# waldstein94/Stratified-Transformer

Measured on AMD Instinct MI355X. Metric: points/sec through StratifiedAttention fwd+bwd, 100k-pt scene, higher is better.
Workload: dtype f32

## Files before the change

### stratified_transformer_amd/csrc/cell_attn.hip

```cpp
#include "cell_common.h"

namespace p2 {


typedef unsigned short bf16_t;
__device__ __forceinline__ float4 ld_row4(const float *p) { return *reinterpret_cast<const float4 *>(p); }
__device__ __forceinline__ float4 ld_row4(const bf16_t *p) {
    const uint2 u = *reinterpret_cast<const uint2 *>(p);
    return make_float4(__uint_as_float(u.x << 16), __uint_as_float(u.x & 0xffff0000u), __uint_as_float(u.y << 16), __uint_as_float(u.y & 0xffff0000u));
}
__device__ __forceinline__ float ld_elem(const float *p) { return *p; }
__device__ __forceinline__ float ld_elem(const bf16_t *p) { return __uint_as_float((unsigned)*p << 16); }
template <typename T>
__device__ __forceinline__ void stage_table_t(T *lds, const T *__restrict__ tab, int L, int h, int head) {
    const int total = 3 * L * 16;
    for (int x = threadIdx.x; x < total; x += blockDim.x) {
        const int i = x % 16, r = (x / 16) % L, ax = x / (16 * L);
        lds[x] = tab[(((size_t)r * h + head) * 16 + i) * 3 + ax];
    }
}

template <int LCAP>
struct TabGeo {
    static constexpr int TS = 3 * LCAP * 16;
    static constexpr size_t bytes(size_t elem) { return (size_t)3 * TS * elem; }
};
struct RowOff {
    int o0, o1, o2;
};
__device__ __forceinline__ RowOff row_off(unsigned w, int L, int c) {
    RowOff r;
    r.o0 = (int)(w & 255u) * 16 + 4 * c;
    r.o1 = (int)(L + ((w >> 8) & 255u)) * 16 + 4 * c;
    r.o2 = (int)(2 * L + ((w >> 16) & 255u)) * 16 + 4 * c;
    return r;
}
template <int OFF>
__device__ __forceinline__ float4 tsum_at(const float *lds, RowOff r) {
    return add4(add4(*reinterpret_cast<const float4 *>(lds + OFF + r.o0), *reinterpret_cast<const float4 *>(lds + OFF + r.o1)),
                *reinterpret_cast<const float4 *>(lds + OFF + r.o2));
}

struct Rows3 {
    float4 a, b, c;
};
template <int OFF, typename T>
__device__ __forceinline__ Rows3 rows_at(const T *lds, RowOff r) {
    Rows3 x;
    x.a = ld_row4(lds + OFF + r.o0);
    x.b = ld_row4(lds + OFF + r.o1);
    x.c = ld_row4(lds + OFF + r.o2);
    return x;
}
typedef float f32x2c __attribute__((ext_vector_type(2)));
__device__ __forceinline__ float4 padd4(float4 a, float4 b) {
    const f32x2c lo = f32x2c{a.x, a.y} + f32x2c{b.x, b.y}, hi = f32x2c{a.z, a.w} + f32x2c{b.z, b.w};
    return make_float4(lo.x, lo.y, hi.x, hi.y);
}
__device__ __forceinline__ float4 pfma4(float s, float4 a, float4 acc) {
    const f32x2c ss = f32x2c{s, s};
    const f32x2c lo = __builtin_elementwise_fma(ss, f32x2c{a.x, a.y}, f32x2c{acc.x, acc.y});
    const f32x2c hi = __builtin_elementwise_fma(ss, f32x2c{a.z, a.w}, f32x2c{acc.z, acc.w});
    return make_float4(lo.x, lo.y, hi.x, hi.y);
}
__device__ __forceinline__ float4 rsum(Rows3 r) { return padd4(padd4(r.a, r.b), r.c); }
__device__ __forceinline__ f32x2c pdot_acc(float4 a, float4 b, f32x2c acc) {
    acc = __builtin_elementwise_fma(f32x2c{a.x, a.y}, f32x2c{b.x, b.y}, acc);
    return __builtin_elementwise_fma(f32x2c{a.z, a.w}, f32x2c{b.z, b.w}, acc);
}
__device__ __forceinline__ float pdot4(float4 a, float4 b) {
    const f32x2c r = pdot_acc(a, b, f32x2c{0.f, 0.f});
    return r.x + r.y;
}

template <int NPMAX, typename F>
__device__ __forceinline__ void dispatch_passes(int np, F f) {
    if (np <= 2) f(std::integral_constant<int, 2>{});
    else if (np == 3) f(std::integral_constant<int, 3>{});
    else if (np == 4 || NPMAX <= 4) f(std::integral_constant<int, 4>{});
    else if constexpr (NPMAX > 4) {
        if (np <= 6) f(std::integral_constant<int, 6>{});
        else f(std::integral_constant<int, 8>{});
    }
}

template <typename T>
struct LaneCtx {
    const T *lds;
    int L, lane, p, c, head, h, C, hoff;
};
struct CellBufs {
    rsrc_t rel, key, qid;
};

template <int NPA, typename T>
__device__ __forceinline__ void load_key_rows(const LaneCtx<T> &x, const CellBufs &cb, const T *__restrict__ rows, int j0, float4 (&r4)[NPA]) {
    unsigned keys[NPA];
    bload_words<NPA>(cb.key, (j0 + x.p * NPA) * 4, keys);
#pragma unroll
    for (int t = 0; t < NPA; t++) r4[t] = ld_row4(rows + (size_t)keys[t] * x.C + x.hoff);
}

template <int NPA, int TS, typename T>
__device__ __forceinline__ void fwd_sweep_logits(const LaneCtx<T> &x, const CellTask &ct, const CellBufs &cb, rsrc_t rs_p,
                                                 const T *__restrict__ q, const T *__restrict__ k, float *__restrict__ ml,
                                                 int ch, bool single, int j0, int nkc) {
    const int p = x.p, c = x.c;
    const int nvalid = min(max(nkc - p * NPA, 0), NPA);
    float4 k4[NPA];
    load_key_rows<NPA, T>(x, cb, k, j0, k4);
    int ids = (int)bload_u32(cb.qid, x.lane * 4);
    int i_nx = __builtin_amdgcn_readlane(ids, 0);
    float4 q4_nx = ld_row4(q + (size_t)i_nx * x.C + x.hoff);
    unsigned w_nx[NPA];
    bload_words<NPA>(cb.rel, (j0 + p * NPA) * 4, w_nx);
    for (int il = 0; il < ct.nq; il++) {
        const int i = i_nx;
        const float4 q4 = q4_nx;
        unsigned w[NPA];
#pragma unroll
        for (int t = 0; t < NPA; t++) w[t] = w_nx[t];
        const int roff = (il * ct.nk + j0 + p * NPA) * 4;
        if (((il + 1) & 63) == 0) ids = (int)bload_u32(cb.qid, (il + 1 + x.lane) * 4);
        i_nx = __builtin_amdgcn_readlane(ids, (il + 1) & 63);
        q4_nx = ld_row4(q + (size_t)i_nx * x.C + x.hoff);
        bload_words<NPA>(cb.rel, roff + ct.nk * 4, w_nx);
        float lg[NPA];
        float mx = -INFINITY;
        RowOff ro = row_off(w[0], x.L, c);
        Rows3 rq = rows_at<0, T>(x.lds, ro), rk = rows_at<TS, T>(x.lds, ro);
#pragma unroll
        for (int t = 0; t < NPA; t++) {
            Rows3 rq1 = rq, rk1 = rk;
            if (t + 1 < NPA) {
                ro = row_off(w[t + 1], x.L, c);
                rq1 = rows_at<0, T>(x.lds, ro);
                rk1 = rows_at<TS, T>(x.lds, ro);
            }
            const f32x2c d2 = pdot_acc(k4[t], rsum(rk), pdot_acc(q4, rsum(rq), pdot_acc(q4, k4[t], f32x2c{0.f, 0.f})));
            const float s = quad_sum(d2.x + d2.y);
            lg[t] = (t < nvalid && !(w[t] >> 31)) ? s : -INFINITY;
            mx = fmaxf(mx, lg[t]);
            rq = rq1;
            rk = rk1;
            __builtin_amdgcn_sched_barrier(0);
        }
        mx = slots_max16(mx);
        if (single) {
            float sum = 0.f;
#pragma unroll
            for (int t = 0; t < NPA; t++) {
                lg[t] = __expf(lg[t] - mx);
                sum += lg[t];
            }
            const float inv = 1.0f / slots_sum16(sum);
#pragma unroll
            for (int t = 0; t < NPA; t++) lg[t] *= inv;
            if (c == 0) bstore_floats<NPA>(rs_p, roff, lg, nvalid);
        } else {
            float *st = ml + ((size_t)i * x.h + x.head) * 2;
            const float m_old = ch ? st[0] : -INFINITY, l_old = ch ? st[1] : 0.f;
            const float m_new = fmaxf(m_old, mx);
            float sum = 0.f;
#pragma unroll
            for (int t = 0; t < NPA; t++) sum += __expf(lg[t] - m_new);
            if (c == 0) bstore_floats<NPA>(rs_p, roff, lg, nvalid);
            sum = slots_sum16(sum);
            if (x.lane == 0) {
                st[0] = m_new;
                st[1] = (m_old == -INFINITY ? 0.f : l_old * __expf(m_old - m_new)) + sum;
            }
        }
    }
}

template <int NPA, int TS, typename T>
__device__ __forceinline__ void fwd_sweep_values(const LaneCtx<T> &x, const CellTask &ct, const CellBufs &cb, rsrc_t rs_p,
                                                 const T *__restrict__ v, const float *__restrict__ ml, float *__restrict__ out,
                                                 int ch, bool single, int j0, int nkc) {
    const int p = x.p, c = x.c;
    const int nvalid = min(max(nkc - p * NPA, 0), NPA);
    float4 v4[NPA];
    load_key_rows<NPA, T>(x, cb, v, j0, v4);
    unsigned w_nx[NPA];
    float a_nx[NPA];
    bload_words<NPA>(cb.rel, (j0 + p * NPA) * 4, w_nx);
    bload_floats<NPA>(rs_p, (j0 + p * NPA) * 4, a_nx);
    int ids = (int)bload_u32(cb.qid, x.lane * 4);
    for (int il = 0; il < ct.nq; il++) {
        if (il && (il & 63) == 0) ids = (int)bload_u32(cb.qid, (il + x.lane) * 4);
        const int i = __builtin_amdgcn_readlane(ids, il & 63);
        const int roff = (il * ct.nk + j0 + p * NPA) * 4;
        unsigned w[NPA];
        float a[NPA];
#pragma unroll
        for (int t = 0; t < NPA; t++) {
            w[t] = w_nx[t];
            a[t] = a_nx[t];
        }
        bload_words<NPA>(cb.rel, roff + ct.nk * 4, w_nx);
        bload_floats<NPA>(rs_p, roff + ct.nk * 4, a_nx);
        if (!single) {
            const float *st = ml + ((size_t)i * x.h + x.head) * 2;
            const float m = st[0], inv = 1.0f / st[1];
#pragma unroll
            for (int t = 0; t < NPA; t++) a[t] = __expf(a[t] - m) * inv;
            if (c == 0) bstore_floats<NPA>(rs_p, roff, a, nvalid);
        }
        float4 acc = make_float4(0.f, 0.f, 0.f, 0.f);
        Rows3 rv = rows_at<2 * TS, T>(x.lds, row_off(w[0], x.L, c));
#pragma unroll
        for (int t = 0; t < NPA; t++) {
            Rows3 rv1 = rv;
            if (t + 1 < NPA) rv1 = rows_at<2 * TS, T>(x.lds, row_off(w[t + 1], x.L, c));
            const float at = t < nvalid ? a[t] : 0.f;
            acc = pfma4(at, padd4(rsum(rv), v4[t]), acc);
            rv = rv1;
            __builtin_amdgcn_sched_barrier(0);
        }
        const float4 tot = slots_sum16_4(acc);
        if (p == 0) {
            float *o = out + (size_t)i * x.C + x.hoff;
            stg4(o, ch ? add4(tot, ldg4(o)) : tot);
        }
    }
}

template <int NP, int LCAP, typename T>
__global__ __launch_bounds__(CA_WAVES * 64) void cell_fwd_kernel(pointops2_cell_plan pl, int h, int L, const T *__restrict__ q,
                                                                 const T *__restrict__ k, const T *__restrict__ v,
                                                                 const T *__restrict__ table_q, const T *__restrict__ table_k,
                                                                 const T *__restrict__ table_v, float *__restrict__ out,
                                                                 float *__restrict__ ml, float *__restrict__ pbuf, size_t plane) {
    constexpr int D = 16, TS = TabGeo<LCAP>::TS;
    extern __shared__ float lds_raw[];
    T *lds = reinterpret_cast<T *>(lds_raw);
    LaneCtx<T> x;
    x.lds = lds;
    x.L = L;
    x.h = h;
    x.head = blockIdx.y;
    x.C = h * D;
    x.lane = threadIdx.x & 63;
    x.p = x.lane >> 2;
    x.c = x.lane & 3;
    x.hoff = x.head * D + 4 * x.c;
    const int wave = __builtin_amdgcn_readfirstlane(threadIdx.x >> 6);
    stage_table_t<T>(lds, table_q, L, h, x.head);
    stage_table_t<T>(lds + TS, table_k, L, h, x.head);
    stage_table_t<T>(lds + 2 * TS, table_v, L, h, x.head);
    __syncthreads();
    const int nC = share_count(pl, pl.counts[0]);
    float *pb = pbuf + (size_t)x.head * plane;
    const int slots = gridDim.x * CA_WAVES, slot = blockIdx.x * CA_WAVES + wave;
    for (int round = 0; round * slots < nC; round++) {
        const int task = snake_task(round, slot, slots);
        if (task >= nC) continue;
        const CellTask ct = cell_task(pl, share_task(pl, task));
        const int nch = (ct.nk + 16 * NP - 1) / (16 * NP);
        const unsigned tile_bytes = (unsigned)ct.nq * ct.nk * 4u;
        CellBufs cb;
        cb.rel = make_rsrc(pl.relp + ct.pbase, tile_bytes);
        cb.key = make_rsrc(pl.cell_keys + ct.kb, (unsigned)ct.nk * 4u);
        cb.qid = make_rsrc(pl.cell_order + ct.qs, (unsigned)ct.nq * 4u);
        const rsrc_t rs_p = make_rsrc(pb + ct.pbase, tile_bytes);
        for (int ch = 0; ch < nch; ch++) {
            const int j0 = ch * 16 * NP, nkc = min(16 * NP, ct.nk - j0);
            dispatch_passes<NP>((nkc + 15) >> 4, [&](auto tag) {
                fwd_sweep_logits<decltype(tag)::value, TS, T>(x, ct, cb, rs_p, q, k, ml, ch, nch == 1, j0, nkc);
            });
        }
        for (int ch = 0; ch < nch; ch++) {
            const int j0 = ch * 16 * NP, nkc = min(16 * NP, ct.nk - j0);
            dispatch_passes<NP>((nkc + 15) >> 4, [&](auto tag) {
                fwd_sweep_values<decltype(tag)::value, TS, T>(x, ct, cb, rs_p, v, ml, out, ch, nch == 1, j0, nkc);
            });
        }
    }
}

template <int NPA, typename T>
__device__ __forceinline__ void flush_key_pass(float *scr, float4 acc, rsrc_t rs_key, int j0, int t, int nkc, float *__restrict__ grad,
                                               const LaneCtx<T> &x) {
    *reinterpret_cast<float4 *>(scr + x.p * 16 + 4 * x.c) = acc;
    __builtin_amdgcn_s_waitcnt(0xC07F);
    __builtin_amdgcn_wave_barrier();
#pragma unroll
    for (int kk = 0; kk < 4; kk++) {
        const int s = (x.lane >> 4) + 4 * kk;
        const int jl = s * NPA + t;
        const int key = (int)bload_u32(rs_key, (j0 + jl) * 4);
        if (jl < nkc) unsafeAtomicAdd(grad + (size_t)key * x.C + x.head * 16 + (x.lane & 15), scr[s * 16 + (x.lane & 15)]);
    }
    __builtin_amdgcn_s_waitcnt(0xC07F);
    __builtin_amdgcn_wave_barrier();
}

template <int NPA, int TS, typename T>
__device__ __forceinline__ void bwd_sweep_values(const LaneCtx<T> &x, const CellTask &ct, const CellBufs &cb, rsrc_t rs_p, rsrc_t rs_g,
                                                 float *scr, const float *__restrict__ go, const float *__restrict__ out,
                                                 const T *__restrict__ v, float *__restrict__ grad_v, int j0, int nkc) {
    const int p = x.p, c = x.c;
    const int nvalid = min(max(nkc - p * NPA, 0), NPA);
    float4 v4[NPA], dv4[NPA];
    load_key_rows<NPA, T>(x, cb, v, j0, v4);
#pragma unroll
    for (int t = 0; t < NPA; t++) dv4[t] = make_float4(0.f, 0.f, 0.f, 0.f);
    unsigned w_nx[NPA];
    float a_nx[NPA];
    bload_words<NPA>(cb.rel, (j0 + p * NPA) * 4, w_nx);
    bload_floats<NPA>(rs_p, (j0 + p * NPA) * 4, a_nx);
    int ids = (int)bload_u32(cb.qid, x.lane * 4);
    int i_nx = __builtin_amdgcn_readlane(ids, 0);
    float4 go_nx = ldg4(go + (size_t)i_nx * x.C + x.hoff), o_nx = ldg4(out + (size_t)i_nx * x.C + x.hoff);
    for (int il = 0; il < ct.nq; il++) {
        const int roff = (il * ct.nk + j0 + p * NPA) * 4;
        const float4 go4 = go_nx, o4 = o_nx;
        unsigned w[NPA];
        float a[NPA];
#pragma unroll
        for (int t = 0; t < NPA; t++) {
            w[t] = w_nx[t];
            a[t] = t < nvalid ? a_nx[t] : 0.f;
        }
        if (((il + 1) & 63) == 0) ids = (int)bload_u32(cb.qid, (il + 1 + x.lane) * 4);
        i_nx = __builtin_amdgcn_readlane(ids, (il + 1) & 63);
        go_nx = ldg4(go + (size_t)i_nx * x.C + x.hoff);
        o_nx = ldg4(out + (size_t)i_nx * x.C + x.hoff);
        bload_words<NPA>(cb.rel, roff + ct.nk * 4, w_nx);
        bload_floats<NPA>(rs_p, roff + ct.nk * 4, a_nx);
        const float delta = quad_sum(pdot4(go4, o4));
        float gs[NPA];
        Rows3 rv = rows_at<2 * TS, T>(x.lds, row_off(w[0], x.L, c));
#pragma unroll
        for (int t = 0; t < NPA; t++) {
            Rows3 rv1 = rv;
            if (t + 1 < NPA) rv1 = rows_at<2 * TS, T>(x.lds, row_off(w[t + 1], x.L, c));
            const float ga = quad_sum(pdot4(go4, padd4(rsum(rv), v4[t])));
            gs[t] = a[t] * (ga - delta);
            dv4[t] = pfma4(a[t], go4, dv4[t]);
            rv = rv1;
            __builtin_amdgcn_sched_barrier(0);
        }
        if (c == 0) bstore_floats<NPA>(rs_g, roff, gs, nvalid);
    }
#pragma unroll
    for (int t = 0; t < NPA; t++) flush_key_pass<NPA, T>(scr, dv4[t], cb.key, j0, t, nkc, grad_v, x);
}

template <int NPA, int TS, typename T>
__device__ __forceinline__ void bwd_sweep_keys(const LaneCtx<T> &x, const CellTask &ct, const CellBufs &cb, rsrc_t rs_g, float *scr,
                                               const T *__restrict__ q, const T *__restrict__ k, float *__restrict__ grad_q,
                                               float *__restrict__ grad_k, int ch, int j0, int nkc) {
    const int p = x.p, c = x.c;
    const int nvalid = min(max(nkc - p * NPA, 0), NPA);
    float4 k4[NPA], dk4[NPA];
    load_key_rows<NPA, T>(x, cb, k, j0, k4);
#pragma unroll
    for (int t = 0; t < NPA; t++) dk4[t] = make_float4(0.f, 0.f, 0.f, 0.f);
    unsigned w_nx[NPA];
    float g_nx[NPA];
    bload_words<NPA>(cb.rel, (j0 + p * NPA) * 4, w_nx);
    bload_floats<NPA>(rs_g, (j0 + p * NPA) * 4, g_nx);
    int ids = (int)bload_u32(cb.qid, x.lane * 4);
    int i_nx = __builtin_amdgcn_readlane(ids, 0);
    float4 q_nx = ld_row4(q + (size_t)i_nx * x.C + x.hoff);
    for (int il = 0; il < ct.nq; il++) {
        const int i = i_nx;
        const int roff = (il * ct.nk + j0 + p * NPA) * 4;
        const float4 q4 = q_nx;
        unsigned w[NPA];
        float g[NPA];
#pragma unroll
        for (int t = 0; t < NPA; t++) {
            w[t] = w_nx[t];
            g[t] = t < nvalid ? g_nx[t] : 0.f;
        }
        if (((il + 1) & 63) == 0) ids = (int)bload_u32(cb.qid, (il + 1 + x.lane) * 4);
        i_nx = __builtin_amdgcn_readlane(ids, (il + 1) & 63);
        q_nx = ld_row4(q + (size_t)i_nx * x.C + x.hoff);
        bload_words<NPA>(cb.rel, roff + ct.nk * 4, w_nx);
        bload_floats<NPA>(rs_g, roff + ct.nk * 4, g_nx);
        float4 dq = make_float4(0.f, 0.f, 0.f, 0.f);
        RowOff ro = row_off(w[0], x.L, c);
        Rows3 rq = rows_at<0, T>(x.lds, ro), rk = rows_at<TS, T>(x.lds, ro);
#pragma unroll
        for (int t = 0; t < NPA; t++) {
            Rows3 rq1 = rq, rk1 = rk;
            if (t + 1 < NPA) {
                ro = row_off(w[t + 1], x.L, c);
                rq1 = rows_at<0, T>(x.lds, ro);
                rk1 = rows_at<TS, T>(x.lds, ro);
            }
            dq = pfma4(g[t], padd4(rsum(rq), k4[t]), dq);
            dk4[t] = pfma4(g[t], padd4(rsum(rk), q4), dk4[t]);
            rq = rq1;
            rk = rk1;
            __builtin_amdgcn_sched_barrier(0);
        }
        const float4 tot = slots_sum16_4(dq);
        if (p == 0) {
            float *o = grad_q + (size_t)i * x.C + x.hoff;
            stg4(o, ch ? add4(tot, ldg4(o)) : tot);
        }
    }
#pragma unroll
    for (int t = 0; t < NPA; t++) flush_key_pass<NPA, T>(scr, dk4[t], cb.key, j0, t, nkc, grad_k, x);
}

template <int NP, int LCAP, typename T>
__global__ __launch_bounds__(CA_WAVES_BWD * 64) void cell_bwd_kernel(pointops2_cell_plan pl, int h, int L, const float *__restrict__ go,
                                                                 const T *__restrict__ q, const T *__restrict__ k,
                                                                 const T *__restrict__ v, const float *__restrict__ out,
                                                                 const T *__restrict__ table_q, const T *__restrict__ table_k,
                                                                 const T *__restrict__ table_v, const float *__restrict__ pbuf,
                                                                 float *__restrict__ gsbuf, size_t plane, float *__restrict__ grad_q,
                                                                 float *__restrict__ grad_k, float *__restrict__ grad_v) {
    constexpr int D = 16, TS = TabGeo<LCAP>::TS;
    extern __shared__ float lds_raw[];
    T *lds = reinterpret_cast<T *>(lds_raw);
    LaneCtx<T> x;
    x.lds = lds;
    x.L = L;
    x.h = h;
    x.head = blockIdx.y;
    x.C = h * D;
    x.lane = threadIdx.x & 63;
    x.p = x.lane >> 2;
    x.c = x.lane & 3;
    x.hoff = x.head * D + 4 * x.c;
    const int wave = __builtin_amdgcn_readfirstlane(threadIdx.x >> 6);
    float *scr = reinterpret_cast<float *>(lds + 3 * TS) + wave * 256;
    stage_table_t<T>(lds, table_q, L, h, x.head);
    stage_table_t<T>(lds + TS, table_k, L, h, x.head);
    stage_table_t<T>(lds + 2 * TS, table_v, L, h, x.head);
    __syncthreads();
    const int nC = share_count(pl, pl.counts[0]);
    const float *pb = pbuf + (size_t)x.head * plane;
    float *gb = gsbuf + (size_t)x.head * plane;
    const int slots = gridDim.x * CA_WAVES_BWD, slot = blockIdx.x * CA_WAVES_BWD + wave;
    for (int round = 0; round * slots < nC; round++) {
        const int task = snake_task(round, slot, slots);
        if (task >= nC) continue;
        const CellTask ct = cell_task(pl, share_task(pl, task));
        const int nch = (ct.nk + 16 * NP - 1) / (16 * NP);
        const unsigned tile_bytes = (unsigned)ct.nq * ct.nk * 4u;
        CellBufs cb;
        cb.rel = make_rsrc(pl.relp + ct.pbase, tile_bytes);
        cb.key = make_rsrc(pl.cell_keys + ct.kb, (unsigned)ct.nk * 4u);
        cb.qid = make_rsrc(pl.cell_order + ct.qs, (unsigned)ct.nq * 4u);
        const rsrc_t rs_p = make_rsrc(pb + ct.pbase, tile_bytes);
        const rsrc_t rs_g = make_rsrc(gb + ct.pbase, tile_bytes);
        for (int ch = 0; ch < nch; ch++) {
            const int j0 = ch * 16 * NP, nkc = min(16 * NP, ct.nk - j0);
            dispatch_passes<NP>((nkc + 15) >> 4, [&](auto tag) {
                bwd_sweep_values<decltype(tag)::value, TS, T>(x, ct, cb, rs_p, rs_g, scr, go, out, v, grad_v, j0, nkc);
            });
        }
        for (int ch = 0; ch < nch; ch++) {
            const int j0 = ch * 16 * NP, nkc = min(16 * NP, ct.nk - j0);
            dispatch_passes<NP>((nkc + 15) >> 4, [&](auto tag) {
                bwd_sweep_keys<decltype(tag)::value, TS, T>(x, ct, cb, rs_g, scr, q, k, grad_q, grad_k, ch, j0, nkc);
            });
        }
    }
}

struct CFixScale {
    float mul, inv;
};
__device__ __forceinline__ CFixScale c_row_scale(unsigned maxbits, int n) {
    CFixScale sc;
    if (maxbits >= 0x7f800000u) {
        sc.mul = 0.f;
        sc.inv = __uint_as_float(0x7fc00000u);
        return sc;
    }
    const int E = (int)(maxbits >> 23) - 126;
    const int bits_n = 32 - __clz(max(n, 1));
    const int S = max(-126, min(126, 30 - bits_n - E));
    sc.mul = __uint_as_float((unsigned)(S + 127) << 23);
    sc.inv = __uint_as_float((unsigned)(127 - S) << 23);
    return sc;
}

constexpr int CT_WAVES = 8;

template <int TA>
struct CellTableGeo {
    static constexpr int LP = TA * 16;
    static constexpr int ROW = 3 * LP + 16;
    static constexpr size_t walk_bytes() { return (size_t)CT_WAVES * 4 * ROW * 4; }
    static constexpr size_t sum_bytes() { return (size_t)LP * 48 * 4; }
    static constexpr size_t lds_bytes() { return walk_bytes() > sum_bytes() ? walk_bytes() : sum_bytes(); }
};

template <int TA, bool BYKEY, typename XT>
__device__ __forceinline__ void cell_table_grad_body(const pointops2_cell_plan &pl, int h, int L, const float *__restrict__ wbuf, size_t plane,
                                                     const XT *__restrict__ X, float *__restrict__ grad_table) {
    constexpr int D = 16;
    constexpr int MAXP = BYKEY ? 4 : 8;
    using G = CellTableGeo<TA>;
    extern __shared__ float lds[];
    const int wave = __builtin_amdgcn_readfirstlane(threadIdx.x >> 6), lane = threadIdx.x & 63;
    const int C = h * D, head = blockIdx.y;
    const int p = lane >> 2, c = lane & 3;
    const int kq = lane >> 4, col = lane & 15;
    int *hist = reinterpret_cast<int *>(lds) + wave * 4 * G::ROW;
    const float *wb = wbuf + (size_t)head * plane;

    f32x4c acc[TA][3];
#pragma unroll
    for (int bt = 0; bt < TA; bt++)
#pragma unroll
        for (int ax = 0; ax < 3; ax++) acc[bt][ax] = f32x4c{0.f, 0.f, 0.f, 0.f};
    for (int x = lane; x < 4 * G::ROW; x += 64) hist[x] = 0;

    const int nC = BYKEY ? pl.counts[4] : share_count(pl, pl.counts[0]);
    const int slots = gridDim.x * CT_WAVES, slot = blockIdx.x * CT_WAVES + wave;
    for (int round = 0; round * slots < nC; round++) {
        const int task = snake_task(round, slot, slots);
        if (task >= nC) continue;
        CellTask ct;
        if (BYKEY) {
            const int c0 = __builtin_amdgcn_readfirstlane(pl.parent_first[task]), c1 = __builtin_amdgcn_readfirstlane(pl.parent_first[task + 1]);
            ct.qs = __builtin_amdgcn_readfirstlane(pl.cell_qstart[c0]);
            ct.nq = __builtin_amdgcn_readfirstlane(pl.cell_qstart[c1]) - ct.qs;
            ct.kb = __builtin_amdgcn_readfirstlane(pl.cell_kbase[c0]);
            ct.nk = __builtin_amdgcn_readfirstlane(pl.cell_kbase[c0 + 1]) - ct.kb;
            ct.pbase = __builtin_amdgcn_readfirstlane(pl.cell_pbase[c0]);
        } else {
            ct = cell_task(pl, share_task(pl, task));
        }
        const unsigned tile_bytes = (unsigned)ct.nq * ct.nk * 4u;
        const rsrc_t rs_rel = make_rsrc(pl.relp + ct.pbase, tile_bytes);
        const rsrc_t rs_w = make_rsrc(wb + ct.pbase, tile_bytes);
        const rsrc_t rs_row = BYKEY ? make_rsrc(pl.cell_keys + ct.kb, (unsigned)ct.nk * 4u) : make_rsrc(pl.cell_order + ct.qs, (unsigned)ct.nq * 4u);
        const int nrows = BYKEY ? ct.nk : ct.nq, nent = BYKEY ? ct.nq : ct.nk;
        auto entry_off = [&](int r0, int ent) -> int { return (BYKEY ? ent * ct.nk + r0 + c : (r0 + c) * ct.nk + ent) * 4; };
        auto consume = [&](int r0, int e0, float xv, unsigned (&wr)[MAXP], float (&wt)[MAXP]) {
            const int ne = min(nent - e0, 16 * MAXP);
            const bool row_ok = r0 + c < nrows;
            unsigned mxb = 0u;
#pragma unroll
            for (int t = 0; t < MAXP; t++) {
                const bool live = row_ok && e0 + 16 * t + p < nent && !(wr[t] >> 31);
                wt[t] = live ? wt[t] : 0.f;
                mxb = max(mxb, __float_as_uint(fabsf(wt[t])));
            }
            const CFixScale sc = c_row_scale(wave_max_u32(mxb), ne);
            int *myh = hist + c * G::ROW;
#pragma unroll
            for (int t = 0; t < MAXP; t++) {
                if (16 * t < ne && wt[t] != 0.f) {
                    const int v = __float2int_rn(wt[t] * sc.mul);
                    atomicAdd(&myh[wr[t] & 255u], v);
                    atomicAdd(&myh[G::LP + ((wr[t] >> 8) & 255u)], v);
                    atomicAdd(&myh[2 * G::LP + ((wr[t] >> 16) & 255u)], v);
                }
            }
            __builtin_amdgcn_s_waitcnt(0xC07F);
            __builtin_amdgcn_wave_barrier();
            const float b = xv * sc.inv;
#pragma unroll
            for (int bt = 0; bt < TA; bt++)
#pragma unroll
                for (int ax = 0; ax < 3; ax++) {
                    const float a = (float)__hip_atomic_exchange(&hist[kq * G::ROW + ax * G::LP + bt * 16 + col], 0, __ATOMIC_RELAXED,
                                                                 __HIP_MEMORY_SCOPE_WORKGROUP);
                    acc[bt][ax] = __builtin_amdgcn_mfma_f32_16x16x4f32(a, b, acc[bt][ax], 0, 0, 0);
                }
            __builtin_amdgcn_s_waitcnt(0xC07F);
            __builtin_amdgcn_wave_barrier();
        };
        unsigned wr_n[MAXP];
        float wt_n[MAXP];
#pragma unroll
        for (int t = 0; t < MAXP; t++) {
            wr_n[t] = 0x80000000u;
            wt_n[t] = 0.f;
            if (16 * t < nent) {
                wr_n[t] = bload_u32(rs_rel, entry_off(0, 16 * t + p));
                wt_n[t] = bload_f32(rs_w, entry_off(0, 16 * t + p));
            }
        }
        int pt_n = (int)bload_u32(rs_row, kq * 4);
        float xv_n = ld_elem(X + (size_t)pt_n * C + head * D + col);
        pt_n = (int)bload_u32(rs_row, (4 + kq) * 4);
        for (int r0 = 0; r0 < nrows; r0 += 4) {
            unsigned wr[MAXP];
            float wt[MAXP];
#pragma unroll
            for (int t = 0; t < MAXP; t++) {
                wr[t] = wr_n[t];
                wt[t] = wt_n[t];
            }
            const float xv = r0 + kq < nrows ? xv_n : 0.f;
            xv_n = ld_elem(X + (size_t)pt_n * C + head * D + col);
            pt_n = (int)bload_u32(rs_row, (r0 + 8 + kq) * 4);
#pragma unroll
            for (int t = 0; t < MAXP; t++)
                if (16 * t < nent) {
                    wr_n[t] = bload_u32(rs_rel, entry_off(r0 + 4, 16 * t + p));
                    wt_n[t] = bload_f32(rs_w, entry_off(r0 + 4, 16 * t + p));
                }
            consume(r0, 0, xv, wr, wt);
            for (int e0 = 16 * MAXP; e0 < nent; e0 += 16 * MAXP) {
#pragma unroll
                for (int t = 0; t < MAXP; t++) {
                    wr[t] = bload_u32(rs_rel, entry_off(r0, e0 + 16 * t + p));
                    wt[t] = bload_f32(rs_w, entry_off(r0, e0 + 16 * t + p));
                }
                consume(r0, e0, xv, wr, wt);
            }
        }
    }
    __syncthreads();
    float *sum = lds;
    for (int w = 0; w < CT_WAVES; w++) {
        if (wave == w) {
#pragma unroll
            for (int bt = 0; bt < TA; bt++)
#pragma unroll
                for (int ax = 0; ax < 3; ax++)
#pragma unroll
                    for (int reg = 0; reg < 4; reg++) {
                        float *d = &sum[((bt * 16 + kq * 4 + reg) * 16 + col) * 3 + ax];
                        *d = w ? *d + acc[bt][ax][reg] : acc[bt][ax][reg];
                    }
        }
        __syncthreads();
    }
    for (int x = threadIdx.x; x < L * 48; x += CT_WAVES * 64) {
        const float val = sum[x];
        if (val != 0.f) unsafeAtomicAdd(grad_table + ((size_t)(x / 48) * h + head) * 48 + x % 48, val);
    }
}

template <int TA, typename T>
__global__ __launch_bounds__(CT_WAVES * 64) void cell_table_grad3_kernel(pointops2_cell_plan pl, int h, int L, const float *__restrict__ gsbuf,
                                                                         const float *__restrict__ pbuf, size_t plane,
                                                                         const T *__restrict__ q, const T *__restrict__ k,
                                                                         const float *__restrict__ grad_out, float *__restrict__ gtq,
                                                                         float *__restrict__ gtk, float *__restrict__ gtv) {
    if (blockIdx.z == 0) cell_table_grad_body<TA, true, T>(pl, h, L, gsbuf, plane, k, gtk);
    else if (blockIdx.z == 1) cell_table_grad_body<TA, false, T>(pl, h, L, gsbuf, plane, q, gtq);
    else cell_table_grad_body<TA, false, float>(pl, h, L, pbuf, plane, grad_out, gtv);
}

static int cell_fwd_variant(const pointops2_cell_plan *plan, int h, int hdim, int L, bool bf16, const char **why) {
    *why = nullptr;
    if (plan == nullptr || plan->n_points <= 0) return POINTOPS2_CELL_FWD_NONE;
    if (hdim != 16) { *why = "cell_attention: d != 16"; return POINTOPS2_CELL_FWD_ERROR; }
    if (L < 1) { *why = "cell_attention: no table rows"; return POINTOPS2_CELL_FWD_ERROR; }
    if (L != plan->table_rows) { *why = "cell_attention: the tables' row count differs from the plan's table_rows"; return POINTOPS2_CELL_FWD_ERROR; }
    if (L > 160) { *why = "cell_attention: more than 160 table rows (use the operators)"; return POINTOPS2_CELL_FWD_ERROR; }
    if (L > 80) return POINTOPS2_CELL_FWD_VALU160;
    if (!bf16) {
        const double avg_queries = (double)plan->n_pairs / (double)(plan->n_keyslots > 0 ? plan->n_keyslots : 1);
        if (!((long long)plan->n_points * h >= 96000 && avg_queries < 15.0)) return L <= 64 ? POINTOPS2_CELL_FWD_MFMA64 : POINTOPS2_CELL_FWD_MFMA80;
    }
    return POINTOPS2_CELL_FWD_VALU80;
}

template <typename T>
static void launch_cell_fwd(hipStream_t st, const pointops2_cell_plan *plan, int h, int hdim, int L, const T *q, const T *k, const T *v, const T *table_q,
                            const T *table_k, const T *table_v, float *out, float *ml, float *pbuf) {
    const char *why;
    const int variant = cell_fwd_variant(plan, h, hdim, L, !std::is_same<T, float>::value, &why);
    if (why != nullptr) { set_error(why); return; }
    if (variant == POINTOPS2_CELL_FWD_NONE) return;
    if constexpr (std::is_same<T, float>::value) {
        if (variant == POINTOPS2_CELL_FWD_MFMA64 || variant == POINTOPS2_CELL_FWD_MFMA80) {
            cell_fwd_mfma_launch(st, variant, plan, h, L, q, k, v, table_q, table_k, table_v, out, pbuf);
            check_launch();
            return;
        }
    }
    const dim3 block(CA_WAVES * 64);
    const size_t plane = (size_t)plan->n_pairs;
    if (variant == POINTOPS2_CELL_FWD_VALU80) {
        const size_t lds = TabGeo<80>::bytes(sizeof(T));
        allow_big_lds(cell_fwd_kernel<CA_NP, 80, T>, lds);
        const dim3 grid(cell_grid_x(1, plan->n_cells, h, CA_WAVES), h);
        hipLaunchKernelGGL((cell_fwd_kernel<CA_NP, 80, T>), grid, block, lds, st, *plan, h, L, q, k, v, table_q, table_k, table_v, out, ml,
                           pbuf, plane);
    } else {
        const size_t lds = TabGeo<160>::bytes(sizeof(T));
        allow_big_lds(cell_fwd_kernel<CA_NP, 160, T>, lds);
        const dim3 grid(cell_grid_x(1, plan->n_cells, h, CA_WAVES), h);
        hipLaunchKernelGGL((cell_fwd_kernel<CA_NP, 160, T>), grid, block, lds, st, *plan, h, L, q, k, v, table_q, table_k, table_v, out, ml,
                           pbuf, plane);
    }
    check_launch();
}

template <typename T>
static void launch_cell_bwd(hipStream_t st, const pointops2_cell_plan *plan, int h, int hdim, int L, const float *grad_out, const T *q, const T *k, const T *v,
                            const float *out, const T *table_q, const T *table_k, const T *table_v, const float *pbuf, float *gsbuf, float *grad_q,
                            float *grad_k, float *grad_v, float *grad_table_q, float *grad_table_k, float *grad_table_v) {
    if (plan == nullptr || plan->n_points <= 0) return;
    if (hdim != 16) { set_error("cell_attention: d != 16"); return; }
    if (L < 1 || L > 80) { set_error("cell_attention backward: table rows L must be in 1..80"); return; }
    if (L != plan->table_rows) { set_error("cell_attention backward: the tables' row count differs from the plan's table_rows"); return; }
    const size_t lds = TabGeo<80>::bytes(sizeof(T)) + (size_t)CA_WAVES_BWD * 256 * sizeof(float);
    allow_big_lds(cell_bwd_kernel<CA_NP_BWD, 80, T>, lds);
    const size_t plane = (size_t)plan->n_pairs;
    hipLaunchKernelGGL((cell_bwd_kernel<CA_NP_BWD, 80, T>), dim3(cell_grid_x(1, plan->n_cells, h, CA_WAVES_BWD), h),
                       dim3(CA_WAVES_BWD * 64), lds, st, *plan, h, L, grad_out, q, k, v, out, table_q, table_k, table_v, pbuf, gsbuf, plane, grad_q,
                       grad_k, grad_v);
    const dim3 grid3(cell_grid_x(1, plan->n_cells, h, CT_WAVES), h, 3), tblock(CT_WAVES * 64);
    if (L <= 64) hipLaunchKernelGGL((cell_table_grad3_kernel<4, T>), grid3, tblock, CellTableGeo<4>::lds_bytes(), st, *plan, h, L, gsbuf, pbuf, plane, q, k, grad_out,
                                    grad_table_q, grad_table_k, grad_table_v);
    else hipLaunchKernelGGL((cell_table_grad3_kernel<5, T>), grid3, tblock, CellTableGeo<5>::lds_bytes(), st, *plan, h, L, gsbuf, pbuf, plane, q, k, grad_out,
                            grad_table_q, grad_table_k, grad_table_v);
    check_launch();
}

}

using namespace p2;

extern "C" {

int pointops2_cell_forward_variant(const pointops2_cell_plan *plan, int h, int hdim, int L, int bf16) {
    const char *why;
    return cell_fwd_variant(plan, h, hdim, L, bf16 != 0, &why);
}

void cell_attention_forward_launcher(const pointops2_cell_plan *plan, int h, int hdim, int L, const float *q, const float *k,
                                     const float *v, const float *table_q, const float *table_k, const float *table_v, float *out,
                                     float *ml, float *pbuf) {
    launch_cell_fwd<float>(begin_launch().stream, plan, h, hdim, L, q, k, v, table_q, table_k, table_v, out, ml, pbuf);
}
void cell_attention_backward_launcher(const pointops2_cell_plan *plan, int h, int hdim, int L, const float *grad_out, const float *q,
                                      const float *k, const float *v, const float *out, const float *table_q, const float *table_k,
                                      const float *table_v, const float *pbuf, float *gsbuf, float *grad_q, float *grad_k,
                                      float *grad_v, float *grad_table_q, float *grad_table_k, float *grad_table_v) {
    launch_cell_bwd<float>(begin_launch().stream, plan, h, hdim, L, grad_out, q, k, v, out, table_q, table_k, table_v, pbuf, gsbuf, grad_q, grad_k, grad_v, grad_table_q,
                           grad_table_k, grad_table_v);
}
void cell_attention_forward_bf16_launcher(const pointops2_cell_plan *plan, int h, int hdim, int L, const uint16_t *q, const uint16_t *k,
                                          const uint16_t *v, const uint16_t *table_q, const uint16_t *table_k, const uint16_t *table_v,
                                          float *out, float *ml, float *pbuf) {
    launch_cell_fwd<bf16_t>(begin_launch().stream, plan, h, hdim, L, q, k, v, table_q, table_k, table_v, out, ml, pbuf);
}
void cell_attention_backward_bf16_launcher(const pointops2_cell_plan *plan, int h, int hdim, int L, const float *grad_out, const uint16_t *q,
                                           const uint16_t *k, const uint16_t *v, const float *out, const uint16_t *table_q,
                                           const uint16_t *table_k, const uint16_t *table_v, const float *pbuf, float *gsbuf, float *grad_q,
                                           float *grad_k, float *grad_v, float *grad_table_q, float *grad_table_k, float *grad_table_v) {
    launch_cell_bwd<bf16_t>(begin_launch().stream, plan, h, hdim, L, grad_out, q, k, v, out, table_q, table_k, table_v, pbuf, gsbuf, grad_q, grad_k, grad_v, grad_table_q,
                            grad_table_k, grad_table_v);
}

}
```

### stratified_transformer_amd/csrc/cell_common.h

```cpp
#pragma once
#include "rpe_common.h"
#include <algorithm>

namespace p2 {

typedef float __attribute__((ext_vector_type(4))) f32x4c;

constexpr int CA_NP = 8;
constexpr int CA_NP_BWD = 3;
constexpr int CA_WAVES = 12;
constexpr int CA_WAVES_BWD = 12;

template <int CTRL>
__device__ __forceinline__ float dppf(float v) {
    return __int_as_float(__builtin_amdgcn_update_dpp(0, __float_as_int(v), CTRL, 0xF, 0xF, true));
}
__device__ __forceinline__ float swap16(float v) { return __int_as_float(__builtin_amdgcn_ds_swizzle(__float_as_int(v), 0x401F)); }
__device__ __forceinline__ float quad_sum(float v) {
    v += dppf<0xB1>(v);
    v += dppf<0x4E>(v);
    return v;
}
__device__ __forceinline__ float slots_sum16(float v) {
    v += dppf<0x124>(v);
    v += dppf<0x128>(v);
    v += swap16(v);
    v += __shfl_xor(v, 32, 64);
    return v;
}
__device__ __forceinline__ float slots_max16(float v) {
    v = fmaxf(v, dppf<0x124>(v));
    v = fmaxf(v, dppf<0x128>(v));
    v = fmaxf(v, swap16(v));
    v = fmaxf(v, __shfl_xor(v, 32, 64));
    return v;
}
__device__ __forceinline__ float4 slots_sum16_4(float4 v) {
    return make_float4(slots_sum16(v.x), slots_sum16(v.y), slots_sum16(v.z), slots_sum16(v.w));
}

typedef __amdgpu_buffer_rsrc_t rsrc_t;
__device__ __forceinline__ rsrc_t make_rsrc(const void *base, unsigned bytes) {
    return __builtin_amdgcn_make_buffer_rsrc(const_cast<void *>(base), 0, (int)bytes, 0x00020000);
}
__device__ __forceinline__ unsigned bload_u32(rsrc_t r, int off) { return __builtin_amdgcn_raw_buffer_load_b32(r, off, 0, 0); }
__device__ __forceinline__ float bload_f32(rsrc_t r, int off) { return __uint_as_float(__builtin_amdgcn_raw_buffer_load_b32(r, off, 0, 0)); }
__device__ __forceinline__ void bstore_f32(rsrc_t r, int off, float v) { __builtin_amdgcn_raw_buffer_store_b32(__float_as_uint(v), r, off, 0, 0); }
typedef unsigned u32x2c __attribute__((ext_vector_type(2)));
typedef unsigned u32x3c __attribute__((ext_vector_type(3)));
typedef unsigned u32x4c __attribute__((ext_vector_type(4)));
template <int N>
__device__ __forceinline__ void bload_words(rsrc_t r, int off, unsigned (&w)[N]) {
    static_assert(N == 2 || N == 3 || N == 4 || N == 6 || N == 8, "pass counts of dispatch_passes");
    if constexpr (N == 2) {
        const u32x2c a = __builtin_amdgcn_raw_buffer_load_b64(r, off, 0, 0);
        w[0] = a.x; w[1] = a.y;
    } else if constexpr (N == 3) {
        const u32x3c a = __builtin_amdgcn_raw_buffer_load_b96(r, off, 0, 0);
        w[0] = a.x; w[1] = a.y; w[2] = a.z;
    } else {
        const u32x4c a = __builtin_amdgcn_raw_buffer_load_b128(r, off, 0, 0);
        w[0] = a.x; w[1] = a.y; w[2] = a.z; w[3] = a.w;
        if constexpr (N == 6) {
            const u32x2c b = __builtin_amdgcn_raw_buffer_load_b64(r, off + 16, 0, 0);
            w[4] = b.x; w[5] = b.y;
        } else if constexpr (N == 8) {
            const u32x4c b = __builtin_amdgcn_raw_buffer_load_b128(r, off + 16, 0, 0);
            w[4] = b.x; w[5] = b.y; w[6] = b.z; w[7] = b.w;
        }
    }
}
template <int N>
__device__ __forceinline__ void bload_floats(rsrc_t r, int off, float (&f)[N]) {
    unsigned w[N];
    bload_words<N>(r, off, w);
#pragma unroll
    for (int t = 0; t < N; t++) f[t] = __uint_as_float(w[t]);
}
template <int N>
__device__ __forceinline__ void bstore_floats(rsrc_t r, int off, const float (&f)[N], int nvalid) {
    if (nvalid >= N) {
        if constexpr (N == 2) {
            __builtin_amdgcn_raw_buffer_store_b64(u32x2c{__float_as_uint(f[0]), __float_as_uint(f[1])}, r, off, 0, 0);
        } else if constexpr (N == 3) {
            __builtin_amdgcn_raw_buffer_store_b96(u32x3c{__float_as_uint(f[0]), __float_as_uint(f[1]), __float_as_uint(f[2])}, r, off, 0, 0);
        } else {
            __builtin_amdgcn_raw_buffer_store_b128(u32x4c{__float_as_uint(f[0]), __float_as_uint(f[1]), __float_as_uint(f[2]), __float_as_uint(f[3])}, r,
                                                   off, 0, 0);
            if constexpr (N == 6)
                __builtin_amdgcn_raw_buffer_store_b64(u32x2c{__float_as_uint(f[4]), __float_as_uint(f[5])}, r, off + 16, 0, 0);
            else if constexpr (N == 8)
                __builtin_amdgcn_raw_buffer_store_b128(u32x4c{__float_as_uint(f[4]), __float_as_uint(f[5]), __float_as_uint(f[6]), __float_as_uint(f[7])},
                                                       r, off + 16, 0, 0);
        }
    } else {
#pragma unroll
        for (int t = 0; t < N; t++)
            if (t < nvalid) bstore_f32(r, off + 4 * t, f[t]);
    }
}


struct CellTask {
    int qs, nq, kb, nk, pbase;
};
__device__ __forceinline__ CellTask cell_task(const pointops2_cell_plan &pl, int task) {
    const int cell = __builtin_amdgcn_readfirstlane(pl.task_list != nullptr ? pl.task_list[task] : pl.cell_perm[task]);
    CellTask t;
    t.qs = __builtin_amdgcn_readfirstlane(pl.cell_qstart[cell]);
    t.nq = __builtin_amdgcn_readfirstlane(pl.cell_qstart[cell + 1]) - t.qs;
    t.kb = __builtin_amdgcn_readfirstlane(pl.cell_kbase[cell]);
    t.nk = __builtin_amdgcn_readfirstlane(pl.cell_kbase[cell + 1]) - t.kb;
    t.pbase = __builtin_amdgcn_readfirstlane(pl.cell_pbase[cell]);
    return t;
}
__device__ __forceinline__ int snake_task(int round, int slot, int slots) { return round * slots + ((round & 1) ? slots - 1 - slot : slot); }
__device__ __forceinline__ int share_count(const pointops2_cell_plan &pl, int n) {
    if (pl.task_list != nullptr) return __builtin_amdgcn_readfirstlane(pl.task_count[0]);
    const int step = pl.task_step > 1 ? pl.task_step : 1, first = pl.task_step > 1 ? pl.task_first : 0;
    return n > first ? (n - first + step - 1) / step : 0;
}
__device__ __forceinline__ int share_task(const pointops2_cell_plan &pl, int i) {
    if (pl.task_list != nullptr) return i;
    return pl.task_step > 1 ? pl.task_first + i * pl.task_step : i;
}


static int cell_grid_x(int per_cu, int tasks, int h, int waves) {
    const int cap = max(1, per_cu * usable_cus() / max(h, 1));
    return max(1, min(cap, div_up(tasks, waves)));
}

void cell_fwd_mfma_launch(hipStream_t st, int variant, const pointops2_cell_plan *plan, int h, int L, const float *q, const float *k, const float *v,
                          const float *table_q, const float *table_k, const float *table_v, float *out, float *pbuf);

}
```

Before: 8.838 million.

## Fuse backward value and key sweeps into a single pass per key chunk

The two backward sweeps (values, then keys/queries) are merged into one loop over queries. The gradient scale is computed and used straight away instead of being written to a scratch buffer and read back, which removes one full walk over the query list and its index and row loads. The key-gradient and value-gradient atomic flushes now share one set of key-index loads. Keys per pass for backward drop from 3 to 2, apparently to offset the extra register pressure of holding k, v, dk and dv together, at the cost of more chunks per cell.

```diff
diff --git a/stratified_transformer_amd/csrc/cell_attn.hip b/stratified_transformer_amd/csrc/cell_attn.hip
--- a/stratified_transformer_amd/csrc/cell_attn.hip
+++ b/stratified_transformer_amd/csrc/cell_attn.hip
@@ -75,12 +75,14 @@
 
 template <int NPMAX, typename F>
 __device__ __forceinline__ void dispatch_passes(int np, F f) {
-    if (np <= 2) f(std::integral_constant<int, 2>{});
-    else if (np == 3) f(std::integral_constant<int, 3>{});
-    else if (np == 4 || NPMAX <= 4) f(std::integral_constant<int, 4>{});
-    else if constexpr (NPMAX > 4) {
-        if (np <= 6) f(std::integral_constant<int, 6>{});
-        else f(std::integral_constant<int, 8>{});
+    if (np <= 2 || NPMAX <= 2) f(std::integral_constant<int, 2>{});
+    else if (np == 3 || NPMAX <= 3) f(std::integral_constant<int, 3>{});
+    else if constexpr (NPMAX > 3) {
+        if (np == 4 || NPMAX <= 4) f(std::integral_constant<int, 4>{});
+        else if constexpr (NPMAX > 4) {
+            if (np <= 6) f(std::integral_constant<int, 6>{});
+            else f(std::integral_constant<int, 8>{});
+        }
     }
 }
 
@@ -280,32 +282,50 @@
 }
 
 template <int NPA, typename T>
-__device__ __forceinline__ void flush_key_pass(float *scr, float4 acc, rsrc_t rs_key, int j0, int t, int nkc, float *__restrict__ grad,
-                                               const LaneCtx<T> &x) {
-    *reinterpret_cast<float4 *>(scr + x.p * 16 + 4 * x.c) = acc;
-    __builtin_amdgcn_s_waitcnt(0xC07F);
-    __builtin_amdgcn_wave_barrier();
-#pragma unroll
-    for (int kk = 0; kk < 4; kk++) {
-        const int s = (x.lane >> 4) + 4 * kk;
-        const int jl = s * NPA + t;
-        const int key = (int)bload_u32(rs_key, (j0 + jl) * 4);
-        if (jl < nkc) unsafeAtomicAdd(grad + (size_t)key * x.C + x.head * 16 + (x.lane & 15), scr[s * 16 + (x.lane & 15)]);
-    }
-    __builtin_amdgcn_s_waitcnt(0xC07F);
-    __builtin_amdgcn_wave_barrier();
+__device__ __forceinline__ void flush_key_pass(float *scr, float4 dk, float4 dv, rsrc_t rs_key, int j0, int t, int nkc, float *__restrict__ grad_k,
+                                               float *__restrict__ grad_v, const LaneCtx<T> &x) {
+    int key[4];
+#pragma unroll
+    for (int kk = 0; kk < 4; kk++) key[kk] = (int)bload_u32(rs_key, (j0 + ((x.lane >> 4) + 4 * kk) * NPA + t) * 4);
+#pragma unroll
+    for (int g = 0; g < 2; g++) {
+        *reinterpret_cast<float4 *>(scr + x.p * 16 + 4 * x.c) = g ? dv : dk;
+        __builtin_amdgcn_s_waitcnt(0xC07F);
+        __builtin_amdgcn_wave_barrier();
+        float *grad = g ? grad_v : grad_k;
+#pragma unroll
+        for (int kk = 0; kk < 4; kk++) {
+            const int s = (x.lane >> 4) + 4 * kk;
+            if (s * NPA + t < nkc) unsafeAtomicAdd(grad + (size_t)key[kk] * x.C + x.head * 16 + (x.lane & 15), scr[s * 16 + (x.lane & 15)]);
+        }
+        __builtin_amdgcn_s_waitcnt(0xC07F);
+        __builtin_amdgcn_wave_barrier();
+    }
+}
+
+__device__ __forceinline__ void computed_here(float a, float4 b) { asm volatile("" ::"v"(a), "v"(f32x4c{b.x, b.y, b.z, b.w})); }
+__device__ __forceinline__ void computed_here(float4 a, float4 b) {
+    asm volatile("" ::"v"(f32x4c{a.x, a.y, a.z, a.w}), "v"(f32x4c{b.x, b.y, b.z, b.w}));
 }
 
 template <int NPA, int TS, typename T>
-__device__ __forceinline__ void bwd_sweep_values(const LaneCtx<T> &x, const CellTask &ct, const CellBufs &cb, rsrc_t rs_p, rsrc_t rs_g,
-                                                 float *scr, const float *__restrict__ go, const float *__restrict__ out,
-                                                 const T *__restrict__ v, float *__restrict__ grad_v, int j0, int nkc) {
+__device__ __forceinline__ void bwd_sweep(const LaneCtx<T> &x, const CellTask &ct, const CellBufs &cb, rsrc_t rs_p, rsrc_t rs_g, float *scr,
+                                          const float *__restrict__ go, const float *__restrict__ out, const T *__restrict__ q,
+                                          const T *__restrict__ k, const T *__restrict__ v, float *__restrict__ grad_q, float *__restrict__ grad_k,
+                                          float *__restrict__ grad_v, int ch, int j0, int nkc) {
     const int p = x.p, c = x.c;
     const int nvalid = min(max(nkc - p * NPA, 0), NPA);
-    float4 v4[NPA], dv4[NPA];
-    load_key_rows<NPA, T>(x, cb, v, j0, v4);
-#pragma unroll
-    for (int t = 0; t < NPA; t++) dv4[t] = make_float4(0.f, 0.f, 0.f, 0.f);
+    float4 k4[NPA], v4[NPA], dk4[NPA], dv4[NPA];
+    {
+        unsigned keys[NPA];
+        bload_words<NPA>(cb.key, (j0 + p * NPA) * 4, keys);
+#pragma unroll
+        for (int t = 0; t < NPA; t++) {
+            k4[t] = ld_row4(k + (size_t)keys[t] * x.C + x.hoff);
+            v4[t] = ld_row4(v + (size_t)keys[t] * x.C + x.hoff);
+            dk4[t] = dv4[t] = make_float4(0.f, 0.f, 0.f, 0.f);
+        }
+    }
     unsigned w_nx[NPA];
     float a_nx[NPA];
     bload_words<NPA>(cb.rel, (j0 + p * NPA) * 4, w_nx);
@@ -313,9 +333,11 @@
     int ids = (int)bload_u32(cb.qid, x.lane * 4);
     int i_nx = __builtin_amdgcn_readlane(ids, 0);
     float4 go_nx = ldg4(go + (size_t)i_nx * x.C + x.hoff), o_nx = ldg4(out + (size_t)i_nx * x.C + x.hoff);
+    float4 q_nx = ld_row4(q + (size_t)i_nx * x.C + x.hoff);
     for (int il = 0; il < ct.nq; il++) {
+        const int i = i_nx;
         const int roff = (il * ct.nk + j0 + p * NPA) * 4;
-        const float4 go4 = go_nx, o4 = o_nx;
+        const float4 go4 = go_nx, o4 = o_nx, q4 = q_nx;
         unsigned w[NPA];
         float a[NPA];
 #pragma unroll
@@ -327,77 +349,36 @@
         i_nx = __builtin_amdgcn_readlane(ids, (il + 1) & 63);
         go_nx = ldg4(go + (size_t)i_nx * x.C + x.hoff);
         o_nx = ldg4(out + (size_t)i_nx * x.C + x.hoff);
+        q_nx = ld_row4(q + (size_t)i_nx * x.C + x.hoff);
         bload_words<NPA>(cb.rel, roff + ct.nk * 4, w_nx);
         bload_floats<NPA>(rs_p, roff + ct.nk * 4, a_nx);
+        RowOff ro = row_off(w[0], x.L, c);
+        Rows3 rv = rows_at<2 * TS, T>(x.lds, ro), rq = rows_at<0, T>(x.lds, ro), rk = rows_at<TS, T>(x.lds, ro);
         const float delta = quad_sum(pdot4(go4, o4));
         float gs[NPA];
-        Rows3 rv = rows_at<2 * TS, T>(x.lds, row_off(w[0], x.L, c));
+        float4 dq = make_float4(0.f, 0.f, 0.f, 0.f);
 #pragma unroll
         for (int t = 0; t < NPA; t++) {
-            Rows3 rv1 = rv;
-            if (t + 1 < NPA) rv1 = rows_at<2 * TS, T>(x.lds, row_off(w[t + 1], x.L, c));
             const float ga = quad_sum(pdot4(go4, padd4(rsum(rv), v4[t])));
             gs[t] = a[t] * (ga - delta);
             dv4[t] = pfma4(a[t], go4, dv4[t]);
-            rv = rv1;
-            __builtin_amdgcn_sched_barrier(0);
-        }
-        if (c == 0) bstore_floats<NPA>(rs_g, roff, gs, nvalid);
-    }
-#pragma unroll
-    for (int t = 0; t < NPA; t++) flush_key_pass<NPA, T>(scr, dv4[t], cb.key, j0, t, nkc, grad_v, x);
-}
-
-template <int NPA, int TS, typename T>
-__device__ __forceinline__ void bwd_sweep_keys(const LaneCtx<T> &x, const CellTask &ct, const CellBufs &cb, rsrc_t rs_g, float *scr,
-                                               const T *__restrict__ q, const T *__restrict__ k, float *__restrict__ grad_q,
-                                               float *__restrict__ grad_k, int ch, int j0, int nkc) {
-    const int p = x.p, c = x.c;
-    const int nvalid = min(max(nkc - p * NPA, 0), NPA);
-    float4 k4[NPA], dk4[NPA];
-    load_key_rows<NPA, T>(x, cb, k, j0, k4);
-#pragma unroll
-    for (int t = 0; t < NPA; t++) dk4[t] = make_float4(0.f, 0.f, 0.f, 0.f);
-    unsigned w_nx[NPA];
-    float g_nx[NPA];
-    bload_words<NPA>(cb.rel, (j0 + p * NPA) * 4, w_nx);
-    bload_floats<NPA>(rs_g, (j0 + p * NPA) * 4, g_nx);
-    int ids = (int)bload_u32(cb.qid, x.lane * 4);
-    int i_nx = __builtin_amdgcn_readlane(ids, 0);
-    float4 q_nx = ld_row4(q + (size_t)i_nx * x.C + x.hoff);
-    for (int il = 0; il < ct.nq; il++) {
-        const int i = i_nx;
-        const int roff = (il * ct.nk + j0 + p * NPA) * 4;
-        const float4 q4 = q_nx;
-        unsigned w[NPA];
-        float g[NPA];
-#pragma unroll
-        for (int t = 0; t < NPA; t++) {
-            w[t] = w_nx[t];
-            g[t] = t < nvalid ? g_nx[t] : 0.f;
-        }
-        if (((il + 1) & 63) == 0) ids = (int)bload_u32(cb.qid, (il + 1 + x.lane) * 4);
-        i_nx = __builtin_amdgcn_readlane(ids, (il + 1) & 63);
-        q_nx = ld_row4(q + (size_t)i_nx * x.C + x.hoff);
-        bload_words<NPA>(cb.rel, roff + ct.nk * 4, w_nx);
-        bload_floats<NPA>(rs_g, roff + ct.nk * 4, g_nx);
-        float4 dq = make_float4(0.f, 0.f, 0.f, 0.f);
-        RowOff ro = row_off(w[0], x.L, c);
-        Rows3 rq = rows_at<0, T>(x.lds, ro), rk = rows_at<TS, T>(x.lds, ro);
-#pragma unroll
-        for (int t = 0; t < NPA; t++) {
-            Rows3 rq1 = rq, rk1 = rk;
+            computed_here(gs[t], dv4[t]);
             if (t + 1 < NPA) {
                 ro = row_off(w[t + 1], x.L, c);
-                rq1 = rows_at<0, T>(x.lds, ro);
-                rk1 = rows_at<TS, T>(x.lds, ro);
-            }
-            dq = pfma4(g[t], padd4(rsum(rq), k4[t]), dq);
-            dk4[t] = pfma4(g[t], padd4(rsum(rk), q4), dk4[t]);
-            rq = rq1;
-            rk = rk1;
+                rv = rows_at<2 * TS, T>(x.lds, ro);
+            }
             __builtin_amdgcn_sched_barrier(0);
-        }
+            const float g = t < nvalid ? gs[t] : 0.f;
+            dq = pfma4(g, padd4(rsum(rq), k4[t]), dq);
+            dk4[t] = pfma4(g, padd4(rsum(rk), q4), dk4[t]);
+            computed_here(dq, dk4[t]);
+            if (t + 1 < NPA) {
+                rq = rows_at<0, T>(x.lds, ro);
+                rk = rows_at<TS, T>(x.lds, ro);
+            }
+            __builtin_amdgcn_sched_barrier(0);
+        }
+        if (c == 0) bstore_floats<NPA>(rs_g, roff, gs, nvalid);
         const float4 tot = slots_sum16_4(dq);
         if (p == 0) {
             float *o = grad_q + (size_t)i * x.C + x.hoff;
@@ -405,7 +386,7 @@
         }
     }
 #pragma unroll
-    for (int t = 0; t < NPA; t++) flush_key_pass<NPA, T>(scr, dk4[t], cb.key, j0, t, nkc, grad_k, x);
+    for (int t = 0; t < NPA; t++) flush_key_pass<NPA, T>(scr, dk4[t], dv4[t], cb.key, j0, t, nkc, grad_k, grad_v, x);
 }
 
 template <int NP, int LCAP, typename T>
@@ -454,13 +435,7 @@
         for (int ch = 0; ch < nch; ch++) {
             const int j0 = ch * 16 * NP, nkc = min(16 * NP, ct.nk - j0);
             dispatch_passes<NP>((nkc + 15) >> 4, [&](auto tag) {
-                bwd_sweep_values<decltype(tag)::value, TS, T>(x, ct, cb, rs_p, rs_g, scr, go, out, v, grad_v, j0, nkc);
-            });
-        }
-        for (int ch = 0; ch < nch; ch++) {
-            const int j0 = ch * 16 * NP, nkc = min(16 * NP, ct.nk - j0);
-            dispatch_passes<NP>((nkc + 15) >> 4, [&](auto tag) {
-                bwd_sweep_keys<decltype(tag)::value, TS, T>(x, ct, cb, rs_g, scr, q, k, grad_q, grad_k, ch, j0, nkc);
+                bwd_sweep<decltype(tag)::value, TS, T>(x, ct, cb, rs_p, rs_g, scr, go, out, q, k, v, grad_q, grad_k, grad_v, ch, j0, nkc);
             });
         }
     }
diff --git a/stratified_transformer_amd/csrc/cell_common.h b/stratified_transformer_amd/csrc/cell_common.h
--- a/stratified_transformer_amd/csrc/cell_common.h
+++ b/stratified_transformer_amd/csrc/cell_common.h
@@ -7,7 +7,7 @@
 typedef float __attribute__((ext_vector_type(4))) f32x4c;
 
 constexpr int CA_NP = 8;
-constexpr int CA_NP_BWD = 3;
+constexpr int CA_NP_BWD = 2;
 constexpr int CA_WAVES = 12;
 constexpr int CA_WAVES_BWD = 12;
 
```

New measurement: 8.962 million, median of 6. No clear change (+1.4%).
